# dselivanov/rsparse

Measured on AMD Instinct MI355X. Metric: als_iterations_per_sec, higher is better.
Workload: dtype f32 (Gram products of rows > 512 / <= 32 non-zeros as 2 x fp16 / 3 x bf16 split terms of the fp32 operands, fp32 accumulate; everything else fp32); 1 GPU; WRMF implicit ALS, CG(3), synthetic 10000000x1000000, 500155883 nnz, rank 128, lambda 0.1; survey_config=3, feedback=implicit, n_items=1000000, nnz=500155883, rank=128, solver=conjugate_gradient, cg_steps=3, parallelism=rows sharded x1, factors replicated

## Files before the change

rsparse_amd/build.py:

```python
import subprocess
import sys
import time
from concurrent.futures import ThreadPoolExecutor
from pathlib import Path

PKG = Path(__file__).resolve().parent
CSRC = PKG / "csrc"
SRC = [CSRC / n for n in ("wrmf_kernels.hip", "wrmf_cgq.hip", "wrmf_cgp.hip", "wrmf_ne.hip", "wrmf_chol.hip", "wrmf_chol_wave.hip", "wrmf_chol_mf.hip", "wrmf_cg_mf.hip", "wrmf_chol_lr.hip",
                          "wrmf_topk.hip", "wrmf_topk_large.hip", "wrmf_similar.hip", "wrmf_metrics.hip", "wrmf_hits.hip", "wrmf_lists.hip", "wrmf_diversity.hip", "wrmf_mmr.hip", "wrmf_ranks.hip", "wrmf_score.hip", "wrmf_softals.hip", "wrmf_itemknn.hip", "wrmf_candidates.hip", "wrmf_sample.hip", "wrmf_sample_weighted.hip", "wrmf_split.hip", "wrmf_confidence.hip", "wrmf_events.hip", "wrmf_explain.hip", "wrmf_init.hip", "wrmf_ingest.hip", "wrmf_nnls.hip", "wrmf_bias.hip", "wrmf_lu.hip",
                          "wrmf_f64.hip", "wrmf_wide.hip", "wrmf_wide_cg.hip", "wrmf_ctx_kernels.hip", "wrmf_schedule.cpp", "wrmf_capi.cpp", "wrmf_f64_capi.cpp", "wrmf_capi_host.cpp", "wrmf_ctx.cpp")]
HEADERS = [CSRC / "wrmf_chol_mf.attrs.csv", CSRC / "wrmf_mf.h", CSRC / "wrmf_internal.h", CSRC / "wrmf_capi_common.h", CSRC / "wrmf_schedule.h", CSRC / "wrmf_device.h", CSRC / "wrmf_sample_team.h", CSRC / "wrmf_wave.h", CSRC / "wrmf_csr_rows.h", CSRC / "wrmf_ldlt.h", CSRC / "wrmf_f64.h", CSRC / "wrmf_topk_plan.h", CSRC / "wrmf_ctx_layout.h", PKG.parent / "include" / "rsparse_wrmf_hip.h"]
DEPS = SRC + HEADERS
OUT = PKG / "lib" / "librsparse_wrmf_hip.so"
FLAGS = ["--offload-arch=gfx950", "-O3", "-std=c++17", "-fPIC"]


EXTRA_FLAGS = {n: ["-mllvm", "-forceattrs-csv-path=" + str(CSRC / "wrmf_chol_mf.attrs.csv"), "-fno-slp-vectorize"] for n in ("wrmf_chol_mf.hip", "wrmf_cg_mf.hip")}
AUDITED = {"wrmf_chol_mf.hip", "wrmf_cg_mf.hip"}
REG_LIMIT = {"wrmf_cg_mf.hip": 512}
NO_SPILL = {"wrmf_cgq.hip": ("14als_cgq_kernelILi128ELi24ELi4ELi4E",),
            "wrmf_cgp.hip": ("14als_cgp_kernelILb0ELb1ELi16ELb1E",),
            "wrmf_explain.hip": ("14explain_kernelIfLi128E",),
            "wrmf_sample.hip": ("13sample_kernelILi64E", "13sample_kernelILi256E"),
            "wrmf_sample_weighted.hip": ("22sample_weighted_kernelILi64E", "22sample_weighted_kernelILi256E"),
            "wrmf_hits.hip": ("18hit_metrics_kernelILb0E", "18hit_metrics_kernelILb1E"),
            "wrmf_lists.hip": ("19list_metrics_kernelILb0E", "19list_metrics_kernelILb1E"),
            "wrmf_diversity.hip": ("21list_diversity_kernelI", "21item_inv_norms_kernelI"),
            "wrmf_mmr.hip": ("10mmr_kernelI",),
            "wrmf_confidence.hip": ("conf_moments_kernel", "conf_moments_finish_kernel", "conf_table_kernel", "conf_apply_kernel"),
            "wrmf_events.hip": ("events_pack_kernel", "events_now_kernel", "events_heads_kernel", "events_reduce_kernel",
                                "events_long_chunks_kernel", "events_long_finish_kernel"),
            "wrmf_cg_mf.hip": ("rsparse_hip_als_cg_mf_implicit", "rsparse_hip_als_cg_mf_implicit_any"),
            "wrmf_softals.hip": ("softals_span_kernel", "softals_finish_kernel", "softals_empty_rows_kernel"),
            "wrmf_itemknn.hip": ("knn_scatter_kernel", "knn_mask_kernel", "knn_select_kernel", "knn_gather_kernel", "knn_cand_select_kernel",
                                 "knn_ranks_kernel"),
            "wrmf_split.hip": ("split_count_wave_kernel", "split_count_team_kernel", "split_write_wave_kernel", "split_write_team_kernel")}
RESOURCE_FLAG = "-Rpass-analysis=kernel-resource-usage"


def resource_violations(remarks, patterns, limit=256):
    import re
    rows, cur = [], None
    for line in remarks.splitlines():
        m = re.search(r"remark:\s+(.*?) \[-Rpass", line)
        if not m:
            continue
        t = m.group(1).strip()
        if t.startswith("Function Name:"):
            cur = {"name": t.split(":", 1)[1].strip()}
            rows.append(cur)
        elif ":" in t and cur is not None:
            k, v = t.rsplit(":", 1)
            cur[k.strip()] = v.strip()
    bad = []
    for pat in patterns:
        hit = [r for r in rows if pat in r["name"]]
        if not hit:
            bad.append((pat, "no such kernel in the compilation"))
        for r in hit:
            regs = int(r.get("VGPRs", "0")) + int(r.get("AGPRs", "0"))
            for key in ("VGPRs Spill", "ScratchSize [bytes/lane]"):
                if int(r.get(key, "0")):
                    bad.append((r["name"], "%s = %s" % (key, r[key])))
            if regs > limit:
                bad.append((r["name"], "%d vector registers" % regs))
    return bad


def audit_listing(src, extra, obj):
    sys.path.insert(0, str(PKG.parent / "tools" / "dbg"))
    import acc_audit
    lst = obj.with_suffix(".s")

    def listing(flags, floor):
        cmd = ["hipcc", *FLAGS, *flags, "-S", "--cuda-device-only", str(src), "-o", str(lst)]
        r = subprocess.run(cmd, stdout=subprocess.PIPE, stderr=subprocess.PIPE, text=True)
        if r.returncode != 0:
            raise RuntimeError("hipcc -S failed on %s:\n%s" % (src.name, r.stderr[-3000:]))
        acc, flight, _ = acc_audit.audit(str(lst), quiet=True, acc_floor=floor)
        return acc, flight, lst.read_text()
    acc, flight, text = listing(extra, 0)
    import re
    nfree = re.findall(r"\.amdhsa_kernel (\w+)[\s\S]*?\.amdhsa_next_free_vgpr (\d+)", text)
    limit = REG_LIMIT.get(src.name, 256)
    two_waves = bool(nfree) and all(int(v) <= limit for name, v in nfree if "_any" not in name)
    if acc == 0 and flight == 0 and two_waves:
        return
    print("  %s: audit of the two-waves-per-SIMD build failed (accumulator-file %d, in-flight %d, layout ok %s): rebuilding with -DMF_SAFE"
          % (src.name, acc, flight, two_waves), flush=True)
    safe = ["-DMF_SAFE"]
    cmd = ["hipcc", *FLAGS, *safe, "-c", str(src), "-o", str(obj)]
    r = subprocess.run(cmd, stdout=subprocess.PIPE, stderr=subprocess.PIPE, text=True)
    if r.returncode != 0:
        raise RuntimeError("hipcc failed on %s (MF_SAFE):\n%s" % (src.name, r.stderr[-3000:]))
    acc, flight, text = listing(safe, 96)
    if acc or flight:
        raise RuntimeError("%s: the MF_SAFE build fails the audit too (accumulator-file %d, in-flight %d)" % (src.name, acc, flight))


def build(force=False, verbose=False, out=None):
    out = Path(out) if out else OUT
    out.parent.mkdir(exist_ok=True)
    objdir = OUT.parent / "obj"
    objdir.mkdir(parents=True, exist_ok=True)
    src = [s for s in SRC if s.exists()]
    hdr_m = max(h.stat().st_mtime for h in HEADERS)
    todo, objs = [], []
    for s in src:
        o = objdir / (s.stem + ".o")
        objs.append(o)
        if force or not o.exists() or o.stat().st_mtime < max(s.stat().st_mtime, hdr_m):
            todo.append((s, o))
    if not todo and out.exists() and all(out.stat().st_mtime >= o.stat().st_mtime for o in objs):
        return out

    def compile_one(so):
        s, o = so
        t0 = time.time()
        extra = EXTRA_FLAGS.get(s.name, [])
        guard = NO_SPILL.get(s.name)
        cmd = ["hipcc", *FLAGS, *extra, *([RESOURCE_FLAG] if guard else []), "-c", str(s), "-o", str(o)]
        r = subprocess.run(cmd, stdout=subprocess.PIPE, stderr=subprocess.PIPE, text=True)
        if r.returncode != 0:
            raise RuntimeError("hipcc failed on %s:\n%s" % (s.name, r.stderr[-6000:]))
        if guard:
            bad = resource_violations(r.stderr, guard, REG_LIMIT.get(s.name, 256))
            if bad:
                o.unlink()
                raise RuntimeError("%s: kernels that must not spill do:\n%s" % (s.name, "\n".join("  %s: %s" % b for b in bad)))
        if s.name in AUDITED:
            audit_listing(s, extra, o)
        if verbose:
            print("  %-20s %.1f s" % (s.name, time.time() - t0), flush=True)

    with ThreadPoolExecutor(max_workers=8) as ex:
        list(ex.map(compile_one, todo))
    cmd = ["hipcc", "--offload-arch=gfx950", "-fPIC", "-shared", *map(str, objs), "-ldl", "-lpthread", "-o", str(out)]
    subprocess.check_call(cmd)
    return out


if __name__ == "__main__":
    argv = sys.argv[1:]
    outp = argv[argv.index("--out") + 1] if "--out" in argv else None
    t0 = time.time()
    print(build(force="--force" in argv, verbose=True, out=outp), "%.1f s" % (time.time() - t0))
```

rsparse_amd/csrc/wrmf_kernels.hip:

```cpp
#include "wrmf_internal.h"
#include "wrmf_device.h"

namespace rsparse_hip {
namespace {

using namespace dev;

template <int KP, int T, int W, bool IMPLICIT>
struct CgSmem {
  static constexpr int LDT = Geo<KP>::LDT;
  static constexpr size_t gram_floats = IMPLICIT ? (size_t)KP * KP : 0;
  static constexpr size_t tile_floats = (size_t)W * T * LDT;
  static constexpr size_t vec_floats = (size_t)W * KP;
  static constexpr size_t red_floats = (size_t)2 * W * KP + 2 * W;
  static constexpr size_t short_bytes = (gram_floats + tile_floats + vec_floats) * 4 + 16;
  static constexpr size_t long_bytes = (gram_floats + tile_floats + vec_floats + red_floats) * 4 + 16;
};

template <int KP, int W>
__device__ __forceinline__ void load_gram_lds(float* sG, const float* __restrict__ G, int k, int tid) {
  for (int e = tid; e < KP * KP; e += W * 64) {
    const int r = e / KP, c = e % KP;
    sG[e] = (r < k && c < k) ? G[(size_t)r * k + c] : 0.f;
  }
}

template <int KP, int T, int W, bool IMPLICIT, bool VEC>
__global__ __launch_bounds__(W * 64) void als_cg_short_kernel(AlsArgs a) {
  constexpr int EPL = Geo<KP>::EPL, LDT = Geo<KP>::LDT;
  extern __shared__ __attribute__((aligned(16))) char smem[];
  float* sG = reinterpret_cast<float*>(smem);
  float* sTiles = sG + CgSmem<KP, T, W, IMPLICIT>::gram_floats;
  float* sVecs = sTiles + CgSmem<KP, T, W, IMPLICIT>::tile_floats;
  int* sCtr = reinterpret_cast<int*>(sVecs + CgSmem<KP, T, W, IMPLICIT>::vec_floats);

  const int tid = threadIdx.x, lane = tid & 63, wv = rfl(tid >> 6);
  const int k = a.k;
  if constexpr (IMPLICIT) load_gram_lds<KP, W>(sG, a.XtX, k, tid);
  for (int e = tid; e < (int)(CgSmem<KP, T, W, IMPLICIT>::tile_floats + CgSmem<KP, T, W, IMPLICIT>::vec_floats);
       e += W * 64)
    sTiles[e] = 0.f;
  if (tid == 0) *sCtr = 0;
  __syncthreads();

  float* tile = sTiles + wv * T * LDT;
  float* vec = sVecs + wv * KP;
  const int row0 = blockIdx.x * kRowsPerWGShort;
  const int row_end = min(a.n_cols, row0 + kRowsPerWGShort);
  const int e0 = lane * EPL;
  const bool active = e0 < KP;
  const int jl = lane % T;
  double wloss = 0.0;
  const bool gb = IMPLICIT && a.gbias != 0.f;
  const float gbias = gb ? a.gbias : 0.f, ltgt = gb ? a.loss_tgt_const : 1.f;

  while (true) {
    int rr = 0;
    if (lane == 0) rr = atomicAdd(sCtr, 1);
    const int row = row0 + rfl(rr);
    if (row >= row_end) break;
    const int p1 = rfl(a.col_ptrs[row]), p2 = rfl(a.col_ptrs[row + 1]);
    const int cnt = p2 - p1;
    if (cnt > T) continue;
    float* yrow = a.Y + (size_t)row * k;
    if (cnt <= 0 && !gb) {
      for (int e = lane; e < k; e += 64) yrow[e] = 0.f;
      continue;
    }
    const bool jvalid = jl < cnt;
    const int myidx = jvalid ? a.row_idx[p1 + jl] : 0;
    const float c = jvalid ? a.vals[p1 + jl] : 0.f;
    wave_sync();
    gather_chunk<KP, T, VEC>(a.X, k, myidx, cnt, tile, lane);

    float x[EPL], r[EPL], p[EPL], ap[EPL];
#pragma unroll
    for (int u = 0; u < EPL; u++) x[u] = (active && e0 + u < k) ? yrow[e0 + u] : 0.f;
    const float lam_use =
        IMPLICIT ? 0.f : (float)(a.lambda_loss * (a.dynamic_lambda ? (double)(float)cnt : 1.0));

    put_vec<KP>(vec, x, lane, active);
    wave_sync();
    float t = tile_dot<KP, T>(tile, vec, lane);
    float wgt = jvalid ? (IMPLICIT ? c - (c - 1.f) * (t + gbias) : c - t) : 0.f;
#pragma unroll
    for (int u = 0; u < EPL; u++) r[u] = 0.f;
    tile_axpy<KP>(tile, wgt, cnt, lane, active, r);
    if constexpr (IMPLICIT) {
      gram_mv<KP>(sG, vec, 0, KP, lane, active, -1.f, r);
      if (gb) {
#pragma unroll
        for (int u = 0; u < EPL; u++) r[u] += (active && e0 + u < k) ? a.rhs_init[e0 + u] : 0.f;
      }
    } else {
#pragma unroll
      for (int u = 0; u < EPL; u++) r[u] -= lam_use * x[u];
    }
    float rs = 0.f;
#pragma unroll
    for (int u = 0; u < EPL; u++) { p[u] = r[u]; rs = fmaf(r[u], r[u], rs); }
    float rsold = wave_sum(rs);

    for (int it = 0; it < a.cg_steps; ++it) {
      wave_sync();
      put_vec<KP>(vec, p, lane, active);
      wave_sync();
      t = tile_dot<KP, T>(tile, vec, lane);
      wgt = jvalid ? (IMPLICIT ? (c - 1.f) * t : t) : 0.f;
#pragma unroll
      for (int u = 0; u < EPL; u++) ap[u] = 0.f;
      tile_axpy<KP>(tile, wgt, cnt, lane, active, ap);
      if constexpr (IMPLICIT) {
        gram_mv<KP>(sG, vec, 0, KP, lane, active, 1.f, ap);
      } else {
#pragma unroll
        for (int u = 0; u < EPL; u++) ap[u] = fmaf(lam_use, p[u], ap[u]);
      }
      float pap = 0.f;
#pragma unroll
      for (int u = 0; u < EPL; u++) pap = fmaf(p[u], ap[u], pap);
      pap = wave_sum(pap);
      const float alpha = (float)((double)rsold / (double)pap);
      rs = 0.f;
#pragma unroll
      for (int u = 0; u < EPL; u++) {
        x[u] = fmaf(alpha, p[u], x[u]);
        r[u] = fmaf(-alpha, ap[u], r[u]);
        rs = fmaf(r[u], r[u], rs);
      }
      const float rsnew = wave_sum(rs);
      if (rsnew < kCgTol) break;
      const float beta = (float)((double)rsnew / (double)rsold);
#pragma unroll
      for (int u = 0; u < EPL; u++) p[u] = fmaf(p[u], beta, r[u]);
      rsold = rsnew;
    }

    wave_sync();
    put_vec<KP>(vec, x, lane, active);
    wave_sync();
    t = tile_dot<KP, T>(tile, vec, lane);
    const float d = IMPLICIT ? ltgt - t : c - t;
    const float lj = (jvalid && lane < T) ? (IMPLICIT ? c * d * d : d * d) : 0.f;
    const float rl = wave_sum(lj);
    float xx = 0.f;
#pragma unroll
    for (int u = 0; u < EPL; u++) xx = fmaf(x[u], x[u], xx);
    xx = wave_sum(xx);
    wloss += IMPLICIT ? (double)rl + a.lambda_loss * (double)xx : (double)(rl + lam_use * xx);
#pragma unroll
    for (int u = 0; u < EPL; u++)
      if (active && e0 + u < k) yrow[e0 + u] = x[u];
  }
  if (lane == 0) a.loss_partials[(size_t)blockIdx.x * W + wv] = wloss;
}

template <int KP, int T, int W, bool IMPLICIT, bool VEC>
__global__ __launch_bounds__(W * 64) void als_cg_long_kernel(AlsArgs a, size_t loss_slot0) {
  constexpr int EPL = Geo<KP>::EPL, LDT = Geo<KP>::LDT;
  static_assert(KP % (4 * W) == 0, "Gramian k-range must split evenly over the waves");
  extern __shared__ __attribute__((aligned(16))) char smem[];
  float* sG = reinterpret_cast<float*>(smem);
  float* sTiles = sG + CgSmem<KP, T, W, IMPLICIT>::gram_floats;
  float* sVecs = sTiles + CgSmem<KP, T, W, IMPLICIT>::tile_floats;
  float* sRed = sVecs + CgSmem<KP, T, W, IMPLICIT>::vec_floats;
  float* sRedL = sRed + 2 * W * KP;

  const int tid = threadIdx.x, lane = tid & 63, wv = rfl(tid >> 6);
  const int k = a.k;
  if constexpr (IMPLICIT) load_gram_lds<KP, W>(sG, a.XtX, k, tid);
  for (int e = tid; e < (int)(CgSmem<KP, T, W, IMPLICIT>::tile_floats + CgSmem<KP, T, W, IMPLICIT>::vec_floats +
                              CgSmem<KP, T, W, IMPLICIT>::red_floats);
       e += W * 64)
    sTiles[e] = 0.f;
  __syncthreads();

  float* tile = sTiles + wv * T * LDT;
  float* vec = sVecs + wv * KP;
  const int e0 = lane * EPL;
  const bool active = e0 < KP;
  const int jl = lane % T;
  int buf = 0;
  double wloss = 0.0;
  const bool gb = IMPLICIT && a.gbias != 0.f;
  const float gbias = gb ? a.gbias : 0.f, ltgt = gb ? a.loss_tgt_const : 1.f;

  for (int li = blockIdx.x; li < a.n_long; li += gridDim.x) {
    const int row = rfl(a.long_rows[li]);
    const int p1 = rfl(a.col_ptrs[row]), p2 = rfl(a.col_ptrs[row + 1]);
    const int cnt = p2 - p1;
    const int nchunks = (cnt + T - 1) / T;
    const bool resident = nchunks <= W;
    float* yrow = a.Y + (size_t)row * k;
    const float lam_use =
        IMPLICIT ? 0.f : (float)(a.lambda_loss * (a.dynamic_lambda ? (double)(float)cnt : 1.0));

    int ccnt = 0, cidx = 0;
    float cval = 0.f;
    if (resident && wv < nchunks) {
      const int base = p1 + wv * T;
      ccnt = min(T, p2 - base);
      cidx = jl < ccnt ? a.row_idx[base + jl] : 0;
      cval = jl < ccnt ? a.vals[base + jl] : 0.f;
      wave_sync();
      gather_chunk<KP, T, VEC>(a.X, k, cidx, ccnt, tile, lane);
      wave_sync();
    }

    float x[EPL], r[EPL], p[EPL], ap[EPL];
#pragma unroll
    for (int u = 0; u < EPL; u++) x[u] = (active && e0 + u < k) ? yrow[e0 + u] : 0.f;

    auto sweep = [&](const float(&v)[EPL], const int mode, float(&out)[EPL], float& loss_out) {
      wave_sync();
      put_vec<KP>(vec, v, lane, active);
      wave_sync();
      float acc[EPL];
#pragma unroll
      for (int u = 0; u < EPL; u++) acc[u] = 0.f;
      float lacc = 0.f;
      for (int ch = wv; ch < nchunks; ch += W) {
        if (!resident) {
          const int base = p1 + ch * T;
          ccnt = min(T, p2 - base);
          cidx = jl < ccnt ? a.row_idx[base + jl] : 0;
          cval = jl < ccnt ? a.vals[base + jl] : 0.f;
          wave_sync();
          gather_chunk<KP, T, VEC>(a.X, k, cidx, ccnt, tile, lane);
          wave_sync();
        }
        const bool jvalid = jl < ccnt;
        const float t = tile_dot<KP, T>(tile, vec, lane);
        if (mode == 2) {
          const float d = IMPLICIT ? ltgt - t : cval - t;
          lacc += (jvalid && lane < T) ? (IMPLICIT ? cval * d * d : d * d) : 0.f;
        } else {
          float wgt;
          if (mode == 0) wgt = IMPLICIT ? cval - (cval - 1.f) * (t + gbias) : cval - t;
          else wgt = IMPLICIT ? (cval - 1.f) * t : t;
          wgt = jvalid ? wgt : 0.f;
          tile_axpy<KP>(tile, wgt, ccnt, lane, active, acc);
        }
      }
      float* red = sRed + buf * W * KP;
      if (mode == 2) {
        lacc = wave_sum(lacc);
        if (lane == 0) sRedL[buf * W + wv] = lacc;
      } else {
        if constexpr (IMPLICIT)
          gram_mv<KP>(sG, vec, wv * (KP / W), (wv + 1) * (KP / W), lane, active, mode == 0 ? -1.f : 1.f, acc);
        put_vec<KP>(red + wv * KP, acc, lane, active);
      }
      __syncthreads();
      if (mode == 2) {
        float s = 0.f;
#pragma unroll
        for (int w2 = 0; w2 < W; w2++) s += sRedL[buf * W + w2];
        loss_out = s;
      } else {
#pragma unroll
        for (int u = 0; u < EPL; u++) out[u] = 0.f;
#pragma unroll
        for (int w2 = 0; w2 < W; w2++) {
          if constexpr (EPL == 2) {
            const float2 q = *reinterpret_cast<const float2*>(red + w2 * KP + lane * 2);
            out[0] += q.x;
            out[1] += q.y;
          } else {
            out[0] += active ? red[w2 * KP + lane] : 0.f;
          }
        }
        if constexpr (!IMPLICIT) {
#pragma unroll
          for (int u = 0; u < EPL; u++) out[u] = fmaf(mode == 0 ? -lam_use : lam_use, v[u], out[u]);
        } else if (gb && mode == 0) {
#pragma unroll
          for (int u = 0; u < EPL; u++) out[u] += (active && e0 + u < k) ? a.rhs_init[e0 + u] : 0.f;
        }
      }
      buf ^= 1;
    };

    float dummy = 0.f;
    sweep(x, 0, r, dummy);
    float rs = 0.f;
#pragma unroll
    for (int u = 0; u < EPL; u++) { p[u] = r[u]; rs = fmaf(r[u], r[u], rs); }
    float rsold = wave_sum(rs);
    for (int it = 0; it < a.cg_steps; ++it) {
      sweep(p, 1, ap, dummy);
      float pap = 0.f;
#pragma unroll
      for (int u = 0; u < EPL; u++) pap = fmaf(p[u], ap[u], pap);
      pap = wave_sum(pap);
      const float alpha = (float)((double)rsold / (double)pap);
      rs = 0.f;
#pragma unroll
      for (int u = 0; u < EPL; u++) {
        x[u] = fmaf(alpha, p[u], x[u]);
        r[u] = fmaf(-alpha, ap[u], r[u]);
        rs = fmaf(r[u], r[u], rs);
      }
      const float rsnew = wave_sum(rs);
      if (rsnew < kCgTol) break;
      const float beta = (float)((double)rsnew / (double)rsold);
#pragma unroll
      for (int u = 0; u < EPL; u++) p[u] = fmaf(p[u], beta, r[u]);
      rsold = rsnew;
    }
    float rl = 0.f;
    sweep(x, 2, ap, rl);
    float xx = 0.f;
#pragma unroll
    for (int u = 0; u < EPL; u++) xx = fmaf(x[u], x[u], xx);
    xx = wave_sum(xx);
    if (wv == 0) {
      wloss += IMPLICIT ? (double)rl + a.lambda_loss * (double)xx : (double)(rl + lam_use * xx);
#pragma unroll
      for (int u = 0; u < EPL; u++)
        if (active && e0 + u < k) yrow[e0 + u] = x[u];
    }
  }
  if (tid == 0) a.loss_partials[loss_slot0 + blockIdx.x] = wloss;
}


template <int KP>
__global__ __launch_bounds__(256, 2) void gramian_partial_kernel(const float* __restrict__ X, int k, int64_t n,
                                                              float* __restrict__ partials,
                                                              unsigned* __restrict__ absmax_bits) {
  constexpr int NT = KP / 32, U = 4;
  const int lane = threadIdx.x & 63;
  const int64_t gw = (int64_t)blockIdx.x * 4 + (threadIdx.x >> 6), nw = (int64_t)gridDim.x * 4;
  const int col = lane & 31, half = lane >> 5;
  f32x16 acc[NT][NT];
#pragma unroll
  for (int i = 0; i < NT; i++)
#pragma unroll
    for (int j = 0; j < NT; j++)
#pragma unroll
      for (int e = 0; e < 16; e++) acc[i][j][e] = 0.f;

  float amax = 0.f;
  auto fetch = [&](const int64_t n0, float (&dst)[U][NT]) {
#pragma unroll
    for (int u = 0; u < U; u++) {
      const int64_t ent = n0 + 2 * u + half;
      const int64_t er = ent < n ? ent : n - 1;
#pragma unroll
      for (int mt = 0; mt < NT; mt++) dst[u][mt] = X[er * k + min(mt * 32 + col, k - 1)];
    }
  };
  auto take = [&](const int64_t n0, const float (&src)[U][NT], float (&dst)[U][NT]) {
#pragma unroll
    for (int u = 0; u < U; u++) {
      const bool in = n0 + 2 * u + half < n;
#pragma unroll
      for (int mt = 0; mt < NT; mt++) dst[u][mt] = src[u][mt] * ((in && mt * 32 + col < k) ? 1.f : 0.f);
    }
  };
  float av[U][NT], nx[U][NT];
  const int64_t stride = nw * 2 * U;
  int64_t n0 = gw * 2 * U;
  if (n0 < n) {
    fetch(n0, nx);
    take(n0, nx, av);
  }
  for (; n0 < n; n0 += stride) {
    const bool more = n0 + stride < n;
    if (more) fetch(n0 + stride, nx);
#pragma unroll
    for (int u = 0; u < U; u++)
#pragma unroll
      for (int mt = 0; mt < NT; mt++) amax = fmaxf(amax, fabsf(av[u][mt]));
#pragma unroll
    for (int u = 0; u < U; u++)
#pragma unroll
      for (int mt = 0; mt < NT; mt++)
#pragma unroll
        for (int nt = 0; nt <= mt; nt++)
          acc[mt][nt] = __builtin_amdgcn_mfma_f32_32x32x2f32(av[u][mt], av[u][nt], acc[mt][nt], 0, 0, 0);
    if (more) take(n0 + stride, nx, av);
  }
  if (absmax_bits) {
#pragma unroll
    for (int off = 32; off > 0; off >>= 1) amax = fmaxf(amax, __shfl_xor(amax, off));
    if (lane == 0) atomicMax(absmax_bits, __float_as_uint(amax < 3.0e38f ? amax : 3.0e38f));
  }
  float* out = partials + (size_t)gw * KP * KP;
#pragma unroll
  for (int mt = 0; mt < NT; mt++)
#pragma unroll
    for (int nt = 0; nt <= mt; nt++)
#pragma unroll
      for (int e = 0; e < 16; e++) {
        const int rr = mt * 32 + (e & 3) + 8 * (e >> 2) + 4 * half;
        out[(size_t)rr * KP + nt * 32 + col] = acc[mt][nt][e];
      }
}

constexpr int kGramRedWaves = 16;
__global__ __launch_bounds__(64 * kGramRedWaves) void gramian_reduce_kernel(const float* __restrict__ partials, int nparts, int KP, int k,
                                                                            float ridge, float* __restrict__ G, double* __restrict__ diag) {
  __shared__ double sh[kGramRedWaves][64];
  const int lane = threadIdx.x & 63, wv = threadIdx.x >> 6;
  const int e = blockIdx.x * 64 + lane;
  const bool in = e < k * k;
  const int ee = in ? e : 0;
  const int aa = ee / k, bb = ee % k;
  const int ta = aa / 32, tb = bb / 32;
  const int rr = ta >= tb ? aa : bb, cc = ta >= tb ? bb : aa;
  const int per = (nparts + kGramRedWaves - 1) / kGramRedWaves;
  const int w0 = min(wv * per, nparts), w1 = min(w0 + per, nparts);
  double s = 0.0;
  const float* src = partials + (size_t)rr * KP + cc;
#pragma unroll 8
  for (int w = w0; w < w1; w++) s += (double)src[(size_t)w * KP * KP];
  sh[wv][lane] = s;
  __syncthreads();
  if (wv != 0 || !in) return;
  double t[kGramRedWaves];
#pragma unroll
  for (int w = 0; w < kGramRedWaves; w++) t[w] = sh[w][lane];
#pragma unroll
  for (int m = 1; m < kGramRedWaves; m *= 2)
#pragma unroll
    for (int w = 0; w < kGramRedWaves; w += 2 * m) t[w] += t[w + m];
  s = t[0];
  G[(size_t)bb * k + aa] = (float)s + (aa == bb ? ridge : 0.f);
  if (aa == bb) diag[aa] = s;
}

__global__ void trace_kernel(const double* __restrict__ diag, int k, double* __restrict__ out) {
  if (threadIdx.x == 0 && blockIdx.x == 0) {
    double s = 0.0;
    for (int i = 0; i < k; i++) s += diag[i];
    *out = s;
  }
}

__global__ __launch_bounds__(256) void weighted_sumsq_kernel(const float* __restrict__ X, int k, int64_t n,
                                                             const float* __restrict__ w, double* __restrict__ partials) {
  __shared__ double sh[4];
  const int64_t total = n * k;
  double s = 0.0;
  for (int64_t e = (int64_t)blockIdx.x * 256 + threadIdx.x; e < total; e += (int64_t)gridDim.x * 256) {
    const float v = X[e];
    const float wj = w ? w[e / k] : 1.f;
    s += (double)(v * v * wj);
  }
  for (int m = 32; m >= 1; m >>= 1) s += __shfl_xor(s, m);
  if ((threadIdx.x & 63) == 0) sh[threadIdx.x >> 6] = s;
  __syncthreads();
  if (threadIdx.x == 0) partials[blockIdx.x] = (sh[0] + sh[1]) + (sh[2] + sh[3]);
}

__global__ __launch_bounds__(256) void sum_partials_kernel(const double* __restrict__ partials, size_t n,
                                                           double* __restrict__ out) {
  __shared__ double sh[4];
  double s = 0.0;
  for (size_t e = threadIdx.x; e < n; e += 256) s += partials[e];
  for (int m = 32; m >= 1; m >>= 1) s += __shfl_xor(s, m);
  if ((threadIdx.x & 63) == 0) sh[threadIdx.x >> 6] = s;
  __syncthreads();
  if (threadIdx.x == 0) *out = (sh[0] + sh[1]) + (sh[2] + sh[3]);
}

__global__ __launch_bounds__(256) void sum_partials_stage_kernel(const double* __restrict__ partials, size_t n,
                                                                 double* __restrict__ tail) {
  __shared__ double sh[4];
  const size_t per = (n + gridDim.x - 1) / gridDim.x, lo = (size_t)blockIdx.x * per, hi = lo + per < n ? lo + per : n;
  double s = 0.0;
  for (size_t e = lo + threadIdx.x; e < hi; e += 256) s += partials[e];
  for (int m = 32; m >= 1; m >>= 1) s += __shfl_xor(s, m);
  if ((threadIdx.x & 63) == 0) sh[threadIdx.x >> 6] = s;
  __syncthreads();
  if (threadIdx.x == 0) tail[blockIdx.x] = (sh[0] + sh[1]) + (sh[2] + sh[3]);
}

__global__ void f64_to_f32_kernel(const double* __restrict__ in, float* __restrict__ out, size_t n) {
  for (size_t e = (size_t)blockIdx.x * blockDim.x + threadIdx.x; e < n; e += (size_t)gridDim.x * blockDim.x)
    out[e] = (float)in[e];
}
__global__ void f32_to_f64_kernel(const float* __restrict__ in, double* __restrict__ out, size_t n) {
  for (size_t e = (size_t)blockIdx.x * blockDim.x + threadIdx.x; e < n; e += (size_t)gridDim.x * blockDim.x)
    out[e] = (double)in[e];
}

template <typename K>
hipError_t set_lds(K kernel, size_t bytes) {
  return hipFuncSetAttribute(reinterpret_cast<const void*>(kernel), hipFuncAttributeMaxDynamicSharedMemorySize,
                             (int)bytes);
}

template <int KP, bool IMPLICIT, bool VEC>
hipError_t launch_cg_t(const AlsArgs& a, hipStream_t s, hipEvent_t* ev) {
  constexpr int T = kTileNnz, W = kWavesPerWG;
  using SM = CgSmem<KP, T, W, IMPLICIT>;
  hipError_t err;
  const int grid_s = (a.n_cols + kRowsPerWGShort - 1) / kRowsPerWGShort;
  if (ev && (err = hipEventRecord(ev[0], s)) != hipSuccess) return err;
  if (grid_s > 0) {
    auto ks = als_cg_short_kernel<KP, T, W, IMPLICIT, VEC>;
    if ((err = set_lds(ks, SM::short_bytes)) != hipSuccess) return err;
    prof_note(ev, reinterpret_cast<const void*>(ks));
    hipLaunchKernelGGL(ks, dim3(grid_s), dim3(W * 64), SM::short_bytes, s, a);
    if ((err = hipGetLastError()) != hipSuccess) return err;
  }
  if (ev && (err = hipEventRecord(ev[1], s)) != hipSuccess) return err;
  if (a.n_long > 0) {
    const int grid_l = (a.n_long + kRowsPerWGLong - 1) / kRowsPerWGLong;
    auto kl = als_cg_long_kernel<KP, T, W, IMPLICIT, VEC>;
    if ((err = set_lds(kl, SM::long_bytes)) != hipSuccess) return err;
    prof_note(ev ? ev + 1 : nullptr, reinterpret_cast<const void*>(kl));
    hipLaunchKernelGGL(kl, dim3(grid_l), dim3(W * 64), SM::long_bytes, s, a, (size_t)grid_s * W);
    if ((err = hipGetLastError()) != hipSuccess) return err;
  }
  if (ev && (err = hipEventRecord(ev[2], s)) != hipSuccess) return err;
  return hipSuccess;
}

}

int padded_rank(int k) {
  if (k <= 0) return 0;
  if (k <= 32) return 32;
  if (k <= 64) return 64;
  if (k <= 128) return 128;
  return 0;
}

size_t cg_loss_slots(int n_cols, int n_long) {
  const size_t grid_s = ((size_t)n_cols + kRowsPerWGShort - 1) / kRowsPerWGShort;
  const size_t grid_l = ((size_t)n_long + kRowsPerWGLong - 1) / kRowsPerWGLong;
  return grid_s * kWavesPerWG + grid_l;
}

size_t chol_loss_slots(int n_cols) {
  return (size_t)(n_cols < kCholMaxGrid ? (n_cols > 0 ? n_cols : 1) : kCholMaxGrid);
}

hipError_t launch_als_cg(const AlsArgs& a, bool implicit, hipStream_t s, hipEvent_t* ev) {
  const int KP = padded_rank(a.k);
  const bool vec = (a.k % 4 == 0) && ((reinterpret_cast<uintptr_t>(a.X) & 15) == 0);
#define RSP_DISPATCH(KPV)                                                             \
  if (KP == KPV) {                                                                    \
    if (implicit) return vec ? launch_cg_t<KPV, true, true>(a, s, ev) : launch_cg_t<KPV, true, false>(a, s, ev); \
    return vec ? launch_cg_t<KPV, false, true>(a, s, ev) : launch_cg_t<KPV, false, false>(a, s, ev);             \
  }
  RSP_DISPATCH(32)
  RSP_DISPATCH(64)
  RSP_DISPATCH(128)
#undef RSP_DISPATCH
  return hipErrorInvalidValue;
}

hipError_t launch_sum_partials(const double* partials, size_t n, double* out, hipStream_t s, double* tail) {
  if (tail && n > 16384) {
    hipLaunchKernelGGL(sum_partials_stage_kernel, dim3(kSumStageBlocks), dim3(256), 0, s, partials, n, tail);
    hipError_t err = hipGetLastError();
    if (err != hipSuccess) return err;
    hipLaunchKernelGGL(sum_partials_kernel, dim3(1), dim3(256), 0, s, tail, (size_t)kSumStageBlocks, out);
    return hipGetLastError();
  }
  hipLaunchKernelGGL(sum_partials_kernel, dim3(1), dim3(256), 0, s, partials, n, out);
  return hipGetLastError();
}

static int gramian_waves(int64_t n) {
  int64_t w = (n + 63) / 64;
  if (w < 1) w = 1;
  if (w > 1024) w = 1024;
  return (int)((w + 3) / 4 * 4);
}

size_t gramian_scratch_floats(int k, int64_t n) {
  const int KP = padded_rank(k);
  return (size_t)gramian_waves(n) * KP * KP + 2 * 128  + 16;
}

hipError_t launch_gramian(const float* X, int k, int64_t n, float ridge, float* XtX, double* sumsq,
                          float* scratch, hipStream_t s, hipEvent_t* ev, unsigned* absmax_bits) {
  const int KP = padded_rank(k);
  if (!KP) return hipErrorInvalidValue;
  const int waves = gramian_waves(n);
  float* partials = scratch;
  double* diag = reinterpret_cast<double*>(scratch + (((size_t)waves * KP * KP + 1) & ~(size_t)1));
  const int grid = waves / 4;
  if (ev) (void)hipEventRecord(ev[0], s);
  prof_note(ev, KP == 32 ? reinterpret_cast<const void*>(gramian_partial_kernel<32>)
                         : (KP == 64 ? reinterpret_cast<const void*>(gramian_partial_kernel<64>)
                                     : reinterpret_cast<const void*>(gramian_partial_kernel<128>)));
  prof_note(ev ? ev + 1 : nullptr, reinterpret_cast<const void*>(gramian_reduce_kernel));
  if (KP == 32) hipLaunchKernelGGL(gramian_partial_kernel<32>, dim3(grid), dim3(256), 0, s, X, k, n, partials, absmax_bits);
  else if (KP == 64) hipLaunchKernelGGL(gramian_partial_kernel<64>, dim3(grid), dim3(256), 0, s, X, k, n, partials, absmax_bits);
  else hipLaunchKernelGGL(gramian_partial_kernel<128>, dim3(grid), dim3(256), 0, s, X, k, n, partials, absmax_bits);
  hipError_t err = hipGetLastError();
  if (err != hipSuccess) return err;
  if (ev) (void)hipEventRecord(ev[1], s);
  hipLaunchKernelGGL(gramian_reduce_kernel, dim3((k * k + 63) / 64), dim3(64 * kGramRedWaves), 0, s, partials, waves, KP, k,
                     ridge, XtX, diag);
  if ((err = hipGetLastError()) != hipSuccess) return err;
  if (sumsq) {
    hipLaunchKernelGGL(trace_kernel, dim3(1), dim3(64), 0, s, diag, k, sumsq);
    err = hipGetLastError();
  }
  if (ev) (void)hipEventRecord(ev[2], s);
  return err;
}

hipError_t launch_weighted_sumsq(const float* X, int k, int64_t n, const float* w, double* out, double* scratch,
                                 hipStream_t s) {
  int64_t blocks = (n * k + 256 * 16 - 1) / (256 * 16);
  if (blocks < 1) blocks = 1;
  if (blocks > 1024) blocks = 1024;
  hipLaunchKernelGGL(weighted_sumsq_kernel, dim3((int)blocks), dim3(256), 0, s, X, k, n, w, scratch);
  hipError_t err = hipGetLastError();
  if (err != hipSuccess) return err;
  return launch_sum_partials(scratch, (size_t)blocks, out, s);
}

hipError_t launch_f64_to_f32(const double* in, float* out, size_t n, hipStream_t s) {
  if (!n) return hipSuccess;
  size_t blocks = (n + 1023) / 1024;
  if (blocks > 4096) blocks = 4096;
  hipLaunchKernelGGL(f64_to_f32_kernel, dim3((int)blocks), dim3(256), 0, s, in, out, n);
  return hipGetLastError();
}
hipError_t launch_f32_to_f64(const float* in, double* out, size_t n, hipStream_t s) {
  if (!n) return hipSuccess;
  size_t blocks = (n + 1023) / 1024;
  if (blocks > 4096) blocks = 4096;
  hipLaunchKernelGGL(f32_to_f64_kernel, dim3((int)blocks), dim3(256), 0, s, in, out, n);
  return hipGetLastError();
}

}
```

Measured before the change: 8.796 iterations/s.

## Compute Gramian partials with split-bf16 MFMA instead of fp32 MFMA

The Gramian partial kernel drops the fp32 32x32x2 MFMA and uses a three-term bf16 split (high/mid/low) with the 32x32x16 bf16 MFMA, keeping six cross products per off-diagonal tile. Diagonal tiles use a symmetric cross accumulator that is transposed through shared memory and added back. The load loop is now double-buffered with a full-tile fast path and hand-placed sched_group_barrier interleaving, and launch bounds go to one block per CU with a larger register limit. The goal is higher matrix-core throughput on the Gram product, at the cost of a small accuracy change and lower occupancy.

Result: no change. 8.831 iterations/s, median of 6 (+0.4%).

```diff
diff --git a/rsparse_amd/build.py b/rsparse_amd/build.py
--- a/rsparse_amd/build.py
+++ b/rsparse_amd/build.py
@@ -17,8 +17,10 @@
 
 EXTRA_FLAGS = {n: ["-mllvm", "-forceattrs-csv-path=" + str(CSRC / "wrmf_chol_mf.attrs.csv"), "-fno-slp-vectorize"] for n in ("wrmf_chol_mf.hip", "wrmf_cg_mf.hip")}
 AUDITED = {"wrmf_chol_mf.hip", "wrmf_cg_mf.hip"}
-REG_LIMIT = {"wrmf_cg_mf.hip": 512}
+REG_LIMIT = {"wrmf_cg_mf.hip": 512,
+             "wrmf_kernels.hip": 512}
 NO_SPILL = {"wrmf_cgq.hip": ("14als_cgq_kernelILi128ELi24ELi4ELi4E",),
+            "wrmf_kernels.hip": ("22gramian_partial_kernelILi32E", "22gramian_partial_kernelILi64E", "22gramian_partial_kernelILi128E"),
             "wrmf_cgp.hip": ("14als_cgp_kernelILb0ELb1ELi16ELb1E",),
             "wrmf_explain.hip": ("14explain_kernelIfLi128E",),
             "wrmf_sample.hip": ("13sample_kernelILi64E", "13sample_kernelILi256E"),
diff --git a/rsparse_amd/csrc/wrmf_kernels.hip b/rsparse_amd/csrc/wrmf_kernels.hip
--- a/rsparse_amd/csrc/wrmf_kernels.hip
+++ b/rsparse_amd/csrc/wrmf_kernels.hip
@@ -1,3 +1,5 @@
+#include <type_traits>
+
 #include "wrmf_internal.h"
 #include "wrmf_device.h"
 
@@ -325,62 +327,136 @@
 }
 
 
+typedef __bf16 bf16x8 __attribute__((ext_vector_type(8)));
+
+__device__ __forceinline__ void gram_split(const float (&x)[8], bf16x8& h, bf16x8& m, bf16x8& l) {
+#pragma unroll
+  for (int j = 0; j < 8; j++) {
+    const __bf16 hj = (__bf16)x[j];
+    const float r1 = x[j] - (float)hj;
+    const __bf16 mj = (__bf16)r1;
+    const float r2 = r1 - (float)mj;
+    h[j] = hj;
+    m[j] = mj;
+    l[j] = (__bf16)r2;
+  }
+}
+
+template <int M>
+__device__ __forceinline__ void gram_interleave() {
+  constexpr int V = (64 + M - 1) / M, L = (8 + M - 1) / M;
+#pragma unroll
+  for (int i = 0; i < M; i++) {
+    __builtin_amdgcn_sched_group_barrier(0x008, 1, 0);
+    __builtin_amdgcn_sched_group_barrier(0x002, V, 0);
+    if (i >= M - 8 / L) __builtin_amdgcn_sched_group_barrier(0x020, L, 0);
+  }
+}
+
 template <int KP>
-__global__ __launch_bounds__(256, 2) void gramian_partial_kernel(const float* __restrict__ X, int k, int64_t n,
+__global__ __launch_bounds__(256, 1) void gramian_partial_kernel(const float* __restrict__ X, int k, int64_t n,
                                                               float* __restrict__ partials,
                                                               unsigned* __restrict__ absmax_bits) {
-  constexpr int NT = KP / 32, U = 4;
-  const int lane = threadIdx.x & 63;
-  const int64_t gw = (int64_t)blockIdx.x * 4 + (threadIdx.x >> 6), nw = (int64_t)gridDim.x * 4;
+  constexpr int NT = KP / 32, R = 8, STEP = 2 * R;
+  __shared__ float tr[4][32 * 33];
+  const int lane = threadIdx.x & 63, wv = rfl(threadIdx.x >> 6);
+  const int64_t gw = (int64_t)blockIdx.x * 4 + wv, nw = (int64_t)gridDim.x * 4;
   const int col = lane & 31, half = lane >> 5;
-  f32x16 acc[NT][NT];
-#pragma unroll
-  for (int i = 0; i < NT; i++)
+  f32x16 acc[NT][NT], cross[NT];
+#pragma unroll
+  for (int i = 0; i < NT; i++) {
 #pragma unroll
     for (int j = 0; j < NT; j++)
 #pragma unroll
       for (int e = 0; e < 16; e++) acc[i][j][e] = 0.f;
+#pragma unroll
+    for (int e = 0; e < 16; e++) cross[i][e] = 0.f;
+  }
 
   float amax = 0.f;
-  auto fetch = [&](const int64_t n0, float (&dst)[U][NT]) {
-#pragma unroll
-    for (int u = 0; u < U; u++) {
-      const int64_t ent = n0 + 2 * u + half;
-      const int64_t er = ent < n ? ent : n - 1;
-#pragma unroll
-      for (int mt = 0; mt < NT; mt++) dst[u][mt] = X[er * k + min(mt * 32 + col, k - 1)];
+  int cidx[NT];
+#pragma unroll
+  for (int mt = 0; mt < NT; mt++) cidx[mt] = min(mt * 32 + col, k - 1);
+  auto fetch = [&](auto whole, const int64_t n0, const int mt, float (&dst)[R][NT]) {
+    const int64_t r0 = n0 + R * half;
+    if constexpr (decltype(whole)::value) {
+      const float* p = X + r0 * KP + col;
+#pragma unroll
+      for (int j = 0; j < R; j++) dst[j][mt] = p[j * KP + mt * 32];
+    } else {
+      const int64_t last = n - 1, rb = r0 < last ? r0 : last;
+      const int room = (int)(last - rb < R ? last - rb : R);
+      const float* p = X + rb * k + cidx[mt];
+#pragma unroll
+      for (int j = 0; j < R; j++) dst[j][mt] = p[min(j, room) * k];
     }
   };
-  auto take = [&](const int64_t n0, const float (&src)[U][NT], float (&dst)[U][NT]) {
-#pragma unroll
-    for (int u = 0; u < U; u++) {
-      const bool in = n0 + 2 * u + half < n;
-#pragma unroll
-      for (int mt = 0; mt < NT; mt++) dst[u][mt] = src[u][mt] * ((in && mt * 32 + col < k) ? 1.f : 0.f);
-    }
+  auto prepare = [&](auto whole, const int64_t n0, const int mt, const float (&src)[R][NT], bf16x8 (&op)[3][NT]) {
+    float v[R];
+    const int64_t r0 = n0 + R * half;
+    const int have = (mt * 32 + col < k) ? (int)(n - r0 > R ? R : (n - r0 < 0 ? 0 : n - r0)) : 0;
+#pragma unroll
+    for (int j = 0; j < R; j++) {
+      if constexpr (decltype(whole)::value) v[j] = src[j][mt];
+      else v[j] = src[j][mt] * (j < have ? 1.f : 0.f);
+      amax = fmaxf(amax, fabsf(v[j]));
+    }
+    gram_split(v, op[0][mt], op[1][mt], op[2][mt]);
   };
-  float av[U][NT], nx[U][NT];
-  const int64_t stride = nw * 2 * U;
-  int64_t n0 = gw * 2 * U;
+  float raw[2][R][NT];
+  bf16x8 op[3][NT];
+  const int64_t stride = nw * STEP;
+  int64_t n0 = gw * STEP;
+  auto step = [&](auto whole, auto parity) {
+    constexpr int p = decltype(parity)::value;
+    const bf16x8(&h)[NT] = op[0], (&m)[NT] = op[1], (&l)[NT] = op[2];
+    prepare(whole, n0, 0, raw[p], op);
+    fetch(whole, n0 + 2 * stride, 0, raw[p]);
+    __builtin_amdgcn_sched_barrier(0);
+#pragma unroll
+    for (int mt = 0; mt < NT; mt++) {
+      if (mt + 1 < NT) {
+        prepare(whole, n0, mt + 1, raw[p], op);
+        fetch(whole, n0 + 2 * stride, mt + 1, raw[p]);
+      }
+#pragma unroll
+      for (int nt = 0; nt < mt; nt++) {
+        f32x16 c = acc[mt][nt];
+        c = __builtin_amdgcn_mfma_f32_32x32x16_bf16(m[mt], m[nt], c, 0, 0, 0);
+        c = __builtin_amdgcn_mfma_f32_32x32x16_bf16(l[mt], h[nt], c, 0, 0, 0);
+        c = __builtin_amdgcn_mfma_f32_32x32x16_bf16(h[mt], l[nt], c, 0, 0, 0);
+        c = __builtin_amdgcn_mfma_f32_32x32x16_bf16(m[mt], h[nt], c, 0, 0, 0);
+        c = __builtin_amdgcn_mfma_f32_32x32x16_bf16(h[mt], m[nt], c, 0, 0, 0);
+        acc[mt][nt] = __builtin_amdgcn_mfma_f32_32x32x16_bf16(h[mt], h[nt], c, 0, 0, 0);
+      }
+      acc[mt][mt] = __builtin_amdgcn_mfma_f32_32x32x16_bf16(m[mt], m[mt], acc[mt][mt], 0, 0, 0);
+      acc[mt][mt] = __builtin_amdgcn_mfma_f32_32x32x16_bf16(h[mt], h[mt], acc[mt][mt], 0, 0, 0);
+      cross[mt] = __builtin_amdgcn_mfma_f32_32x32x16_bf16(h[mt], l[mt], cross[mt], 0, 0, 0);
+      cross[mt] = __builtin_amdgcn_mfma_f32_32x32x16_bf16(h[mt], m[mt], cross[mt], 0, 0, 0);
+      if (mt + 1 < NT) {
+        if (mt == 0) gram_interleave<4>();
+        else if (mt == 1) gram_interleave<10>();
+        else gram_interleave<16>();
+      }
+      __builtin_amdgcn_sched_barrier(0);
+    }
+    n0 += stride;
+  };
+  constexpr std::false_type kAny{};
+  constexpr std::true_type kWhole{};
   if (n0 < n) {
-    fetch(n0, nx);
-    take(n0, nx, av);
-  }
-  for (; n0 < n; n0 += stride) {
-    const bool more = n0 + stride < n;
-    if (more) fetch(n0 + stride, nx);
-#pragma unroll
-    for (int u = 0; u < U; u++)
-#pragma unroll
-      for (int mt = 0; mt < NT; mt++) amax = fmaxf(amax, fabsf(av[u][mt]));
-#pragma unroll
-    for (int u = 0; u < U; u++)
-#pragma unroll
-      for (int mt = 0; mt < NT; mt++)
-#pragma unroll
-        for (int nt = 0; nt <= mt; nt++)
-          acc[mt][nt] = __builtin_amdgcn_mfma_f32_32x32x2f32(av[u][mt], av[u][nt], acc[mt][nt], 0, 0, 0);
-    if (more) take(n0 + stride, nx, av);
+#pragma unroll
+    for (int mt = 0; mt < NT; mt++) fetch(kAny, n0, mt, raw[0]);
+#pragma unroll
+    for (int mt = 0; mt < NT; mt++) fetch(kAny, n0 + stride, mt, raw[1]);
+  }
+  while (k == KP && n0 + 3 * stride + STEP <= n) {
+    step(kWhole, std::integral_constant<int, 0>{});
+    step(kWhole, std::integral_constant<int, 1>{});
+  }
+  while (n0 < n) {
+    step(kAny, std::integral_constant<int, 0>{});
+    step(kAny, std::integral_constant<int, 1>{});
   }
   if (absmax_bits) {
 #pragma unroll
@@ -389,14 +465,24 @@
   }
   float* out = partials + (size_t)gw * KP * KP;
 #pragma unroll
-  for (int mt = 0; mt < NT; mt++)
-#pragma unroll
-    for (int nt = 0; nt <= mt; nt++)
+  for (int mt = 0; mt < NT; mt++) {
+#pragma unroll
+    for (int nt = 0; nt < mt; nt++)
 #pragma unroll
       for (int e = 0; e < 16; e++) {
         const int rr = mt * 32 + (e & 3) + 8 * (e >> 2) + 4 * half;
         out[(size_t)rr * KP + nt * 32 + col] = acc[mt][nt][e];
       }
+    __syncthreads();
+#pragma unroll
+    for (int e = 0; e < 16; e++) tr[wv][((e & 3) + 8 * (e >> 2) + 4 * half) * 33 + col] = cross[mt][e];
+    __syncthreads();
+#pragma unroll
+    for (int e = 0; e < 16; e++) {
+      const int r = (e & 3) + 8 * (e >> 2) + 4 * half;
+      out[(size_t)(mt * 32 + r) * KP + mt * 32 + col] = acc[mt][mt][e] + (cross[mt][e] + tr[wv][col * 33 + r]);
+    }
+  }
 }
 
 constexpr int kGramRedWaves = 16;
```
